# HuaiLeiTang/slam_ros

Hardware: NVIDIA B200
Metric: EKF predict+update steps/s at N landmarks (higher is better)
Workload: dtype f64

## Files before the change

slam_ros_b200/csrc/ekf_kernels.cu:

```cuda
#include "ekf_internal.h"
#include "ekf_device.cuh"
#include <stdlib.h>
#include <string.h>
#include <cuda.h>
#include <cooperative_groups.h>
namespace cg = cooperative_groups;

#define EKF_BLOCK 256

namespace {

__device__ __forceinline__ int owner_of_row(const EkfGeom& g, int r) { return (r / EKF_TILE) % g.world; }
__device__ __forceinline__ size_t local_row(const EkfGeom& g, int r) {
  return (size_t)((r / EKF_TILE) / g.world) * EKF_TILE + (size_t)(r % EKF_TILE);
}
__device__ __forceinline__ bool is_hot(int r, int q) {
  return r <= 2 || q == r || (q == r + 1 && (r & 1));
}
__device__ __forceinline__ double hot_value(const EkfGeom& g, const EkfBuffers& b, int r, int q) {
  if (r <= 2) return b.top[(size_t)r * g.ld + q];
  const int j = (r - 3) >> 1;
  if (r & 1) return b.diag[4 * j + (q - r)];
  return b.diag[4 * j + 2];
}
// ... 319 lines not shown
        d.pa = sub_rank2(d.pa, d.v[t], s_ka[i0 + t]);
        d.pb = sub_rank2(d.pb, d.v[t], s_kb[i0 + t]);
      }
    }
  } else if (d.kind == 2) {
    for (int i0 = 0; i0 < npt; i0 += 8) {
      if (i0 > 0) {
#pragma unroll
        for (int t = 0; t < 8; ++t) if (i0 + t < npt) d.v[t] = b.Kp[(size_t)pl.slot(i0 + t) * g.ld + r];
      }
#pragma unroll
      for (int t = 0; t < 8; ++t) if (i0 + t < npt) {
        d.pa = sub_rank2(d.pa, s_ksa[i0 + t], d.v[t]);
        d.pb = sub_rank2(d.pb, s_ksb[i0 + t], d.v[t]);
      }
    }
  }
}
__device__ __forceinline__ void gain_row_emit(const EkfGeom& g, const EkfBuffers& b, const Gate& G, int r, int out_slot,
                                              const GainRow& d) {
  double2 Kr, KSr;
  gain_row(G, d.p0, d.p1, d.p2, d.pa, d.pb, Kr, KSr);
  b.Kp[(size_t)out_slot * g.ld + r] = Kr;
  b.KSp[(size_t)out_slot * g.ld + r] = KSr;
}

__device__ __forceinline__ double* xchg_col(const EkfPeers& pe, const EkfGeom& g, int p, int par, int which) {
  return pe.xchg[p] + ((size_t)(2 * par + which)) * g.ld;
}
__device__ __forceinline__ unsigned long long* xchg_flags(const EkfPeers& pe, const EkfGeom& g, int p) {
  return reinterpret_cast<unsigned long long*>(pe.xchg[p] + (size_t)4 * g.ld);
}
__device__ __forceinline__ unsigned long long ld_acquire_sys(const unsigned long long* p) {
  unsigned long long v;
  asm volatile("ld.acquire.sys.global.u64 %0, [%1];" : "=l"(v) : "l"(p) : "memory");
  return v;
}
__device__ __forceinline__ void st_relaxed_sys(unsigned long long* p, unsigned long long v) {
  asm volatile("st.relaxed.sys.global.u64 [%0], %1;" ::"l"(p), "l"(v) : "memory");
}
__device__ __forceinline__ void xgpu_exchange_barrier(const EkfPeers& pe, const EkfGeom& g, unsigned long long epoch, int* sticky) {
  __threadfence_system();
  for (int p = 0; p < pe.world; ++p) st_relaxed_sys(xchg_flags(pe, g, p) + pe.rank, epoch);
  const unsigned long long* mine = xchg_flags(pe, g, pe.rank);
  for (int q = 0; q < pe.world; ++q) {
    long long spins = 0;
    while (ld_acquire_sys(mine + q) < epoch) {
      if (++spins > 40000000LL) { atomicOr(sticky, EKF_STICKY_XCHG); break; }
    }
  }
}

#ifdef EKF_LINE_TIMING
__device__ unsigned long long g_line_ts[64 * 16];
__device__ __forceinline__ unsigned long long gtimer() { unsigned long long t; asm volatile("mov.u64 %0, %%globaltimer;" : "=l"(t)); return t; }
#define TS(slot) do { if (gtid == 0 && line - line0 < 64) g_line_ts[(line - line0) * 16 + (slot)] = gtimer(); } while (0)
#else
#define TS(slot) do { } while (0)
#endif

template <int FL_THREADS, bool COOP, bool SHARD>
__global__ void __launch_bounds__(FL_THREADS, FL_THREADS == 256 ? 3 : 1) k_scan_lines(EkfGeom g, EkfBuffers b, const double* __restrict__ z,
                                                              const double* __restrict__ R, int line0, int line1,
                                                              int own_slot0, int prev_slot0, const int* __restrict__ prev_cnt_ptr,
                                                              EkfPeers pe) {
  __shared__ int s_min[FL_THREADS / 32];
  __shared__ double2 s_ka[FL_MAXP], s_kb[FL_MAXP], s_ksa[FL_MAXP], s_ksb[FL_MAXP];
  const int prev_cnt = prev_cnt_ptr ? *prev_cnt_ptr : 0;
  EkfDevState* st = b.st;
  const int gtid = blockIdx.x * blockDim.x + threadIdx.x;
  const int gstride = gridDim.x * blockDim.x;
  auto group_sync = [] () {
    if (COOP) cg::this_grid().sync(); else cg::this_cluster().sync();
  };
  const int L = st->L, nl = 3 + 2 * L, epoch = st->epoch, pbase = st->pbase;
  int nm = b.pidx[line0];
  int ne = b.eidx[line0];
  const int xseq0 = SHARD ? st->xseq : 0;
  int xdone = 0;
  double A[3][3], xp[3];
  load_rr(g, b.top, A);
  xp[0] = st->x_pre[0]; xp[1] = st->x_pre[1]; xp[2] = st->x_pre[2];
  bool have_prev = false;
  int np_prev = 0;
  double pv0 = 0.0, pv1 = 0.0;
  double pS[4] = {0, 0, 0, 0};
  for (int line = line0; line <= line1; ++line) {
    const bool gating = line < line1;
    if (!gating && !have_prev) break;
    TS(0);
    double Rl[4] = {0, 0, 0, 0}, z0 = 0, z1 = 0;
    if (gating) {
      Rl[0] = R[4 * line]; Rl[1] = R[4 * line + 1]; Rl[2] = R[4 * line + 2]; Rl[3] = R[4 * line + 3];
      z0 = z[2 * line]; z1 = z[2 * line + 1];
    }
    const double2* Kv = b.Kp + (size_t)(own_slot0 + np_prev) * g.ld;
    const double2* KSv = b.KSp + (size_t)(own_slot0 + np_prev) * g.ld;
    double2 ks[3], kk[3];
    if (have_prev) {
      for (int r = 0; r < 3; ++r) { ks[r] = KSv[r]; kk[r] = Kv[r]; }
    }
    int cand = EKF_NO_MATCH;
    bool robot_done = !have_prev;
    for (int j = gtid; j < L; j += gstride) {
      const int a = 3 + 2 * j, bb = a + 1;
      double t0a = b.top[a], t0b = b.top[bb];
      double t1a = b.top[(size_t)g.ld + a], t1b = b.top[(size_t)g.ld + bb];
      double t2a = b.top[(size_t)2 * g.ld + a], t2b = b.top[(size_t)2 * g.ld + bb];
      double daa = b.diag[4 * j], dab = b.diag[4 * j + 1], dbb = b.diag[4 * j + 2];
      double ya = b.y[a], yb = b.y[bb];
      const int mt = b.matched[j];
      if (have_prev) {
        const double2 ka = Kv[a], kb = Kv[bb], ksa = KSv[a], ksb = KSv[bb];
        t0a = sub_rank2(t0a, ks[0], ka); t0b = sub_rank2(t0b, ks[0], kb);
        t1a = sub_rank2(t1a, ks[1], ka); t1b = sub_rank2(t1b, ks[1], kb);
        t2a = sub_rank2(t2a, ks[2], ka); t2b = sub_rank2(t2b, ks[2], kb);
        daa = sub_rank2(daa, ksa, ka); dab = sub_rank2(dab, ksa, kb); dbb = sub_rank2(dbb, ksb, kb);
        double ta = 0.0, tb = 0.0;
        axpy_skip(ta, ka.x, pv0); axpy_skip(ta, ka.y, pv1);
        axpy_skip(tb, kb.x, pv0); axpy_skip(tb, kb.y, pv1);
        ya = add_rn(ya, ta); yb = add_rn(yb, tb);
        b.top[a] = t0a; b.top[bb] = t0b;
        b.top[(size_t)g.ld + a] = t1a; b.top[(size_t)g.ld + bb] = t1b;
        b.top[(size_t)2 * g.ld + a] = t2a; b.top[(size_t)2 * g.ld + bb] = t2b;
        b.diag[4 * j] = daa; b.diag[4 * j + 1] = dab; b.diag[4 * j + 2] = dbb;
        b.y[a] = ya; b.y[bb] = yb;
      }
// ... 108 lines not shown
        break;
      }
      const double* cA = xchg_col(pe, g, g.rank, xpar, 0);
      const double* cB = xchg_col(pe, g, g.rank, xpar, 1);
      for (r = gtid; r < nl; r += gstride) {
        GainRow e;
        if (r <= 2) { e.p0 = A[r][0]; e.p1 = A[r][1]; e.p2 = A[r][2]; e.pa = b.top[(size_t)r * g.ld + a]; e.pb = b.top[(size_t)r * g.ld + bb]; }
        else {
          e.p0 = b.top[r]; e.p1 = b.top[(size_t)g.ld + r]; e.p2 = b.top[(size_t)2 * g.ld + r];
          if (r == a) { e.pa = b.diag[4 * j]; e.pb = b.diag[4 * j + 1]; }
          else if (r == bb) { e.pa = b.diag[4 * j + 1]; e.pb = b.diag[4 * j + 2]; }
          else { e.pa = __ldcg(cA + r); e.pb = __ldcg(cB + r); }
        }
        gain_row_emit(g, b, G, r, own_slot0 + np, e);
      }
    }
    if (gtid == 0) {
      b.matched[j] = epoch;
      b.jout[line] = j;
      b.pidx[line + 1] = nm + 1; b.eidx[line + 1] = ne;
      st->np = np + 1;
    }
    TS(6);
    group_sync();
    TS(7);
    have_prev = true;
    np_prev = np;
    nm += 1;
    pv0 = G.v[0]; pv1 = G.v[1];
    for (int t = 0; t < 4; ++t) pS[t] = G.S[t];
  }
  if (SHARD && gtid == 0) st->xseq = xseq0 + xdone;
}

struct HotLm { double t0a, t0b, t1a, t1b, t2a, t2b, daa, dab, dbb, ya, yb; int mt; };
__device__ __forceinline__ void hot_load(const EkfGeom& g, const EkfBuffers& b, int j, HotLm& h) {
  const int a = 3 + 2 * j;
  h.t0a = b.top[a]; h.t0b = b.top[a + 1];
  h.t1a = b.top[(size_t)g.ld + a]; h.t1b = b.top[(size_t)g.ld + a + 1];
  h.t2a = b.top[(size_t)2 * g.ld + a]; h.t2b = b.top[(size_t)2 * g.ld + a + 1];
  h.daa = b.diag[4 * j]; h.dab = b.diag[4 * j + 1]; h.dbb = b.diag[4 * j + 2];
  h.ya = b.y[a]; h.yb = b.y[a + 1];
  h.mt = b.matched[j];
}
__device__ __forceinline__ void hot_store(const EkfGeom& g, const EkfBuffers& b, int j, const HotLm& h) {
  const int a = 3 + 2 * j;
  b.top[a] = h.t0a; b.top[a + 1] = h.t0b;
  b.top[(size_t)g.ld + a] = h.t1a; b.top[(size_t)g.ld + a + 1] = h.t1b;
  b.top[(size_t)2 * g.ld + a] = h.t2a; b.top[(size_t)2 * g.ld + a + 1] = h.t2b;
  b.diag[4 * j] = h.daa; b.diag[4 * j + 1] = h.dab; b.diag[4 * j + 2] = h.dbb;
  b.y[a] = h.ya; b.y[a + 1] = h.yb;
}

template <int FL_THREADS, bool COOP, bool CACHED>
__global__ void __launch_bounds__(FL_THREADS, 1) k_scan_lines2(EkfGeom g, EkfBuffers b, const double* __restrict__ z,
                                                               const double* __restrict__ R, int line0, int line1,
                                                               int own_slot0, int prev_slot0, const int* __restrict__ prev_cnt_ptr,
                                                               const double* __restrict__ pred_u, const double* __restrict__ pred_x, int pred_m,
                                                               const int* __restrict__ pred_carry) {
  __shared__ int s_min[FL_THREADS / 32];
  __shared__ double2 s_ka[FL_MAXP], s_kb[FL_MAXP], s_ksa[FL_MAXP], s_ksb[FL_MAXP];
  const int prev_cnt = prev_cnt_ptr ? *prev_cnt_ptr : 0;
  EkfDevState* st = b.st;
  const int gtid = blockIdx.x * blockDim.x + threadIdx.x;
  const int gstride = gridDim.x * blockDim.x;
  const int scribe = gstride - 1;
  auto group_sync = [] () {
    if (COOP) cg::this_grid().sync(); else cg::this_cluster().sync();
  };
  if (pred_u) {
    predict_body(g, b, pred_u, pred_x, pred_m, gtid, gstride, pred_carry);
    __threadfence();
    group_sync();
  }
  const int L = st->L, epoch = st->epoch, pbase = st->pbase;
  int nm = b.pidx[line0];
  int ne = b.eidx[line0];
  double A[3][3], xp[3];
  load_rr(g, b.top, A);
  xp[0] = st->x_pre[0]; xp[1] = st->x_pre[1]; xp[2] = st->x_pre[2];
  constexpr bool cached = CACHED;
  HotLm h;
  if (cached && gtid < L) hot_load(g, b, gtid, h);
  PendingList pl;
  pl.prev_cnt = prev_cnt; pl.prev_slot0 = prev_slot0; pl.own_slot0 = own_slot0;
  for (int line = line0; line < line1; ++line) {
    TS(0);
    const double Rl[4] = {R[4 * line], R[4 * line + 1], R[4 * line + 2], R[4 * line + 3]};
    const double z0 = z[2 * line], z1 = z[2 * line + 1];
    int cand = EKF_NO_MATCH;
    for (int j = gtid; j < L; j += gstride) {
      if (!cached) hot_load(g, b, j, h);
      if (cand == EKF_NO_MATCH && h.mt != epoch) {
        double Cm[5][5];
        for (int r = 0; r < 3; ++r) for (int q = 0; q < 3; ++q) Cm[r][q] = A[r][q];
        Cm[0][3] = Cm[3][0] = h.t0a; Cm[0][4] = Cm[4][0] = h.t0b;
        Cm[1][3] = Cm[3][1] = h.t1a; Cm[1][4] = Cm[4][1] = h.t1b;
        Cm[2][3] = Cm[3][2] = h.t2a; Cm[2][4] = Cm[4][2] = h.t2b;
        Cm[3][3] = h.daa; Cm[3][4] = Cm[4][3] = h.dab; Cm[4][4] = h.dbb;
        Gate G;
        gate_from_block(Cm, h.ya, h.yb, xp, z0, z1, Rl, G);
        if (G.singular) atomicOr(&st->sticky, EKF_STICKY_SINGULAR);
        else if (!gate_rejects_d2(G.d2, g.gate_d2max)) {
          cand = j;
          double* rec = b.gates + (size_t)GATE_REC * j;
          gate_store(rec, G);
          rec[14] = h.t0a; rec[15] = h.t0b; rec[16] = h.t1a; rec[17] = h.t1b; rec[18] = h.t2a; rec[19] = h.t2b;
        }
      }
    }
    TS(1);
    cand = __reduce_min_sync(0xffffffffu, cand);
    if ((threadIdx.x & 31) == 0) s_min[threadIdx.x >> 5] = cand;
    __syncthreads();
    if (threadIdx.x < 32) {
      int v = (threadIdx.x < FL_THREADS / 32) ? s_min[threadIdx.x] : EKF_NO_MATCH;
      v = __reduce_min_sync(0xffffffffu, v);
      if (threadIdx.x == 0 && v != EKF_NO_MATCH) atomicMin(&b.jbest[line], v);
    }
    TS(2);
    group_sync();
    TS(3);
    const int jw = b.jbest[line];
    const int np = nm - pbase;
    if (jw != EKF_NO_MATCH) TS(8);
    if (jw == EKF_NO_MATCH) {
      if (gtid == scribe) { b.ext[ne] = line; b.eidx[line + 1] = ne + 1; b.pidx[line + 1] = nm; b.jout[line] = -1; }
      ne += 1;
      continue;
    }
    const int aw = 3 + 2 * jw, bw = aw + 1;
    const double* rec = b.gates + (size_t)GATE_REC * jw;
    Gate G;
    gate_load(rec, G);
    TS(9);
    const double wt[3][2] = {{rec[14], rec[15]}, {rec[16], rec[17]}, {rec[18], rec[19]}};
    const int npt = prev_cnt + np;
    for (int i = threadIdx.x; i < npt; i += blockDim.x) {
      const int slot = pl.slot(i);
      s_ka[i] = b.Kp[(size_t)slot * g.ld + aw]; s_kb[i] = b.Kp[(size_t)slot * g.ld + bw];
      s_ksa[i] = b.KSp[(size_t)slot * g.ld + aw]; s_ksb[i] = b.KSp[(size_t)slot * g.ld + bw];
    }
    const int out_slot = own_slot0 + np;
    double2 kk[3], ks[3];
#pragma unroll
    for (int r = 0; r < 3; ++r) gain_row(G, A[r][0], A[r][1], A[r][2], wt[r][0], wt[r][1], kk[r], ks[r]);
    if (gtid == scribe) {
#pragma unroll
      for (int r = 0; r < 3; ++r) { b.Kp[(size_t)out_slot * g.ld + r] = kk[r]; b.KSp[(size_t)out_slot * g.ld + r] = ks[r]; }
    }
    TS(10);
    const double v0 = G.v[0], v1 = G.v[1];
    constexpr int CH = 4;
    const int jc = gtid;
    const bool own1 = cached && jc < L;
    double cpa[2] = {0.0, 0.0}, cpb[2] = {0.0, 0.0};
    double2 cv[2][CH];
    int ckind = 0;
    if (own1 && jc != jw) {
      const int a = 3 + 2 * jc;
      ckind = jc < jw ? 1 : 2;
#pragma unroll
      for (int hf = 0; hf < 2; ++hf) {
        const int r = a + hf;
        if (ckind == 1) { cpa[hf] = b.P[(size_t)r * g.ld + aw]; cpb[hf] = b.P[(size_t)r * g.ld + bw]; }
        else { cpa[hf] = b.P[(size_t)aw * g.ld + r]; cpb[hf] = b.P[(size_t)bw * g.ld + r]; }
        const double2* src = ckind == 1 ? b.KSp : b.Kp;
#pragma unroll
        for (int t = 0; t < CH; ++t) if (t < npt) cv[hf][t] = src[(size_t)pl.slot(t) * g.ld + r];
      }
    }
    TS(11);
    __syncthreads();
    TS(4);
    for (int j = gtid; j < L; j += gstride) {
      const int a = 3 + 2 * j, bb = a + 1;
      double2 Ka, KSa, Kb, KSb;
      if (cached) {
        double pa0 = cpa[0], pb0 = cpb[0], pa1 = cpa[1], pb1 = cpb[1];
        if (j == jw) { pa0 = h.daa; pb0 = h.dab; pa1 = h.dab; pb1 = h.dbb; }
        else {
          const double2* src = ckind == 1 ? b.KSp : b.Kp;
          for (int i0 = 0; i0 < npt; i0 += CH) {
            if (i0 > 0) {
#pragma unroll
              for (int t = 0; t < CH; ++t) if (i0 + t < npt) {
                cv[0][t] = src[(size_t)pl.slot(i0 + t) * g.ld + a]; cv[1][t] = src[(size_t)pl.slot(i0 + t) * g.ld + bb];
              }
            }
#pragma unroll
            for (int t = 0; t < CH; ++t) if (i0 + t < npt) {
              if (ckind == 1) {
                pa0 = sub_rank2(pa0, cv[0][t], s_ka[i0 + t]); pb0 = sub_rank2(pb0, cv[0][t], s_kb[i0 + t]);
                pa1 = sub_rank2(pa1, cv[1][t], s_ka[i0 + t]); pb1 = sub_rank2(pb1, cv[1][t], s_kb[i0 + t]);
              } else {
                pa0 = sub_rank2(pa0, s_ksa[i0 + t], cv[0][t]); pb0 = sub_rank2(pb0, s_ksb[i0 + t], cv[0][t]);
                pa1 = sub_rank2(pa1, s_ksa[i0 + t], cv[1][t]); pb1 = sub_rank2(pb1, s_ksb[i0 + t], cv[1][t]);
              }
            }
          }
        }
        TS(12);
        gain_row(G, h.t0a, h.t1a, h.t2a, pa0, pb0, Ka, KSa);
        gain_row(G, h.t0b, h.t1b, h.t2b, pa1, pb1, Kb, KSb);
      } else {
        hot_load(g, b, j, h);
#pragma unroll
        for (int half = 0; half < 2; ++half) {
          const int r = a + half;
          GainRow d;
          d.p0 = half ? h.t0b : h.t0a; d.p1 = half ? h.t1b : h.t1a; d.p2 = half ? h.t2b : h.t2a;
          d.kind = 0;
          if (j == jw) { d.pa = half ? h.dab : h.daa; d.pb = half ? h.dbb : h.dab; }
          else if (j < jw) {
            const double* Pr = b.P + (size_t)r * g.ld;
            d.pa = Pr[aw]; d.pb = Pr[bw];
            d.kind = 1;
#pragma unroll
            for (int t = 0; t < 8; ++t) if (t < npt) d.v[t] = b.KSp[(size_t)pl.slot(t) * g.ld + r];
          } else {
            d.pa = b.P[(size_t)aw * g.ld + r]; d.pb = b.P[(size_t)bw * g.ld + r];
            d.kind = 2;
#pragma unroll
            for (int t = 0; t < 8; ++t) if (t < npt) d.v[t] = b.Kp[(size_t)pl.slot(t) * g.ld + r];
          }
          gain_row_correct(g, b, r, npt, d, pl, s_ka, s_kb, s_ksa, s_ksb);
          if (half) gain_row(G, d.p0, d.p1, d.p2, d.pa, d.pb, Kb, KSb);
          else gain_row(G, d.p0, d.p1, d.p2, d.pa, d.pb, Ka, KSa);
        }
      }
      TS(13);
      b.Kp[(size_t)out_slot * g.ld + a] = Ka; b.KSp[(size_t)out_slot * g.ld + a] = KSa;
      b.Kp[(size_t)out_slot * g.ld + bb] = Kb; b.KSp[(size_t)out_slot * g.ld + bb] = KSb;
      h.t0a = sub_rank2(h.t0a, ks[0], Ka); h.t0b = sub_rank2(h.t0b, ks[0], Kb);
      h.t1a = sub_rank2(h.t1a, ks[1], Ka); h.t1b = sub_rank2(h.t1b, ks[1], Kb);
      h.t2a = sub_rank2(h.t2a, ks[2], Ka); h.t2b = sub_rank2(h.t2b, ks[2], Kb);
      h.daa = sub_rank2(h.daa, KSa, Ka); h.dab = sub_rank2(h.dab, KSa, Kb); h.dbb = sub_rank2(h.dbb, KSb, Kb);
      double ta = 0.0, tb = 0.0;
      axpy_skip(ta, Ka.x, v0); axpy_skip(ta, Ka.y, v1);
      axpy_skip(tb, Kb.x, v0); axpy_skip(tb, Kb.y, v1);
      h.ya = add_rn(h.ya, ta); h.yb = add_rn(h.yb, tb);
      if (j == jw) { h.mt = epoch; b.matched[j] = epoch; }
      hot_store(g, b, j, h);
    }
    TS(5);
    update_robot_block(kk, ks, v0, v1, A, xp);
    if (gtid == scribe) {
      for (int r = 0; r < 3; ++r) {
        for (int q = r; q < 3; ++q) b.top[(size_t)r * g.ld + q] = A[r][q];
        b.y[r] = xp[r]; st->pose[r] = xp[r]; st->x_pre[r] = xp[r];
      }
      st->v[0] = v0; st->v[1] = v1;
      for (int t = 0; t < 4; ++t) st->S[t] = G.S[t];
      b.jout[line] = jw;
      b.pidx[line + 1] = nm + 1; b.eidx[line + 1] = ne;
      st->np = np + 1;
    }
    TS(6);
    nm += 1;
  }
}

__global__ void k_flush_done(EkfBuffers b, int next_line) {
  if (blockIdx.x == 0 && threadIdx.x == 0) { b.st->pbase = b.pidx[next_line]; b.st->np = 0; }
}

__global__ void k_chunk_mark(EkfBuffers b, int next_line, EkfScanView* view) {
  if (blockIdx.x == 0 && threadIdx.x == 0) {
    EkfDevState* st = b.st;
    view->cnt = b.pidx[next_line] - st->pbase; view->L = st->L;
    st->pbase = b.pidx[next_line]; st->np = 0;
  }
}

__global__ void k_queue_all(EkfGeom g, EkfBuffers b, int m) {
  const int gid = blockIdx.x * blockDim.x + threadIdx.x;
  for (int i = gid; i < m; i += gridDim.x * blockDim.x) {
    b.ext[i] = i; b.eidx[i + 1] = i + 1; b.pidx[i + 1] = 0; b.jout[i] = -1;
  }
}

struct TileId { int k, rb, cb; };

__device__ __forceinline__ long long tiles_before(int T, int rank, int world, long long k) {
  return k * (long long)(T - rank) - (long long)world * k * (k - 1) / 2;
}
__device__ __forceinline__ TileId decode_tile(int T, int rank, int world, long long idx) {
  const double A = (double)(T - rank) + 0.5 * world;
  double disc = A * A - 2.0 * world * (double)idx;
  if (disc < 0.0) disc = 0.0;
  long long k = (long long)((A - sqrt(disc)) / world);
  if (k < 0) k = 0;
  while (tiles_before(T, rank, world, k + 1) <= idx) ++k;
  while (k > 0 && tiles_before(T, rank, world, k) > idx) --k;
  TileId t;
  t.k = (int)k;
  t.rb = rank + world * (int)k;
  t.cb = t.rb + (int)(idx - tiles_before(T, rank, world, k));
  return t;
}

template <int C>
__global__ void __launch_bounds__(EKF_BLOCK, 2) k_sweep(EkfGeom g, EkfBuffers b, const int* __restrict__ np_ptr) {
  const int np = np_ptr ? *np_ptr : b.st->np;
  if (np <= 0) return;
  const int nl = 3 + 2 * b.st->L;
  const int T = (nl + EKF_TILE - 1) / EKF_TILE;
  if (g.rank >= T) return;
  const long long K_rows = (T - g.rank + g.world - 1) / g.world;
  const long long total = tiles_before(T, g.rank, g.world, K_rows);
  const long long idx = blockIdx.x;
  if (idx >= total) return;
  const TileId t = decode_tile(T, g.rank, g.world, idx);
// ... 413 lines not shown
    for (int mb = 0; mb < 2; ++mb)
#pragma unroll
      for (int nb = 0; nb < 8; ++nb)
        acc[mb][nb] = *reinterpret_cast<const double2*>(&st.P[(nb * TR + row0 + 8 * mb) * 8 + 2 * tq]);
    if (split) {
      __syncwarp();
      if (lane == 0) mbar_arrive(&sh.emptyP[s]);
    }
    const double* KSw = reinterpret_cast<const double*>(&st.KS[0][0]);
    const double* Kw = reinterpret_cast<const double*>(&st.K[0][0]);
#pragma unroll 2
    for (int k0 = 0; k0 < np; k0 += 2) {
      const int term = k0 + tsel;
      const bool valid = term < np;
      double a[2], bq[8];
#pragma unroll
      for (int mb = 0; mb < 2; ++mb) a[mb] = valid ? -KSw[(term * TR + row0 + 8 * mb) * 2 + comp] : 0.0;
#pragma unroll
      for (int nb = 0; nb < 8; ++nb) bq[nb] = valid ? Kw[(term * TC + 8 * nb + gq) * 2 + comp] : 0.0;
#pragma unroll
      for (int mb = 0; mb < 2; ++mb)
#pragma unroll
        for (int nb = 0; nb < 8; ++nb) dmma884(acc[mb][nb].x, acc[mb][nb].y, a[mb], bq[nb]);
    }
    __syncwarp();
    if (lane == 0) mbar_arrive(&sh.empty[s]);
    double* Pt = dst + ((size_t)lrow0 + row0) * g.ld + (size_t)col0 + 2 * tq;
    if (grow0 + TR <= nl && col0 + TC <= nl) {
#pragma unroll
      for (int mb = 0; mb < 2; ++mb)
#pragma unroll
        for (int nb = 0; nb < 8; ++nb) __stcs(reinterpret_cast<double2*>(Pt + (size_t)(8 * mb) * g.ld + 8 * nb), acc[mb][nb]);
    } else {
#pragma unroll
      for (int mb = 0; mb < 2; ++mb) {
        if (grow0 + row0 + 8 * mb < nl) {
          double* Pr = Pt + (size_t)(8 * mb) * g.ld;
#pragma unroll
          for (int nb = 0; nb < 8; ++nb) {
            const int q = col0 + 8 * nb + 2 * tq;
            if (q + 1 < nl) __stcs(reinterpret_cast<double2*>(Pr + 8 * nb), acc[mb][nb]); else if (q < nl) Pr[8 * nb] = acc[mb][nb].x;
          }
        }
      }
    }
  }
}

__global__ void __launch_bounds__(512) k_end_scan_a(EkfGeom g, EkfBuffers b, const double* __restrict__ z, const double* __restrict__ R, int m,
                                                    int slot0, EkfScanView* view, int prev_slot0, const int* __restrict__ prev_cnt_ptr) {
  EkfDevState* st = b.st;
  __shared__ double s_pose[3];
  __shared__ double s_y01[2];
  if (threadIdx.x == 0) {
    if (m == 0 || b.pidx[m] == 0) {
      b.y[0] = st->x_pre[0]; b.y[1] = st->x_pre[1]; b.y[2] = st->x_pre[2];
      double th = st->x_pre[2];
      normalize_radian(th);
      st->pose[0] = st->x_pre[0]; st->pose[1] = st->x_pre[1]; st->pose[2] = th;
    }
    s_pose[0] = st->pose[0]; s_pose[1] = st->pose[1]; s_pose[2] = st->pose[2];
    s_y01[0] = b.y[0]; s_y01[1] = b.y[1];
  }
  __syncthreads();
  const int ne = b.eidx[m];
  const int L = st->L;
  const int n_add = min(ne, g.cap - L);
  if (threadIdx.x == 0 && blockIdx.x == 0) {
    st->n_added = n_add;
    if (n_add < ne) atomicOr(&st->sticky, EKF_STICKY_CAPACITY);
  }
  {
    const int cnt = b.pidx[m] - st->pbase, r0 = 3 + 2 * L, r1 = 3 + 2 * (L + n_add);
    const int pcnt = prev_cnt_ptr ? *prev_cnt_ptr : 0;
    for (int i = 0; i < cnt + pcnt; ++i) {
      const size_t slot = i < cnt ? slot0 + i : prev_slot0 + (i - cnt);
      for (int r = r0 + threadIdx.x; r < r1; r += blockDim.x) {
        b.Kp[slot * g.ld + r] = make_double2(0.0, 0.0);
        b.KSp[slot * g.ld + r] = make_double2(0.0, 0.0);
      }
    }
  }
  double A[3][3];
  load_rr(g, b.top, A);
  for (int e = blockIdx.x * blockDim.x + threadIdx.x; e < n_add; e += gridDim.x * blockDim.x) {
    const int i = b.ext[e];
    double alfa = z[2 * i], r = z[2 * i + 1];
    const double Rl[4] = {R[4 * i], R[4 * i + 1], R[4 * i + 2], R[4 * i + 3]};
    const int l = 3 + 2 * (L + e);
    r = add_rn(r, add_rn(mul_rn(s_pose[0], cos(alfa)), mul_rn(s_pose[1], sin(alfa))));
    alfa = add_rn(alfa, s_pose[2]);
    double cw, sw;
    cos_sin(alfa, cw, sw);
    const double Gx[2][3] = {{0.0, 0.0, 1.0}, {cw, sw, 0.0}};
    const double Gl[2][2] = {{1.0, 0.0}, {sub_rn(mul_rn(s_y01[1], cw), mul_rn(s_y01[0], sw)), 1.0}};
    normalize_radian(alfa);
    b.y[l] = alfa; b.y[l + 1] = r;
    b.ext_cs[2 * e] = cw; b.ext_cs[2 * e + 1] = sw;
    double GP[2][3] = {{0, 0, 0}, {0, 0, 0}};
    for (int k = 0; k < 3; ++k)
      for (int ii = 0; ii < 2; ++ii) {
        const double t = mul_rn(1.0, Gx[ii][k]);
        if (t != 0.0) for (int jj = 0; jj < 3; ++jj) GP[ii][jj] = add_rn(GP[ii][jj], mul_rn(t, A[k][jj]));
      }
    double Pll[2][2];
    for (int ii = 0; ii < 2; ++ii)
      for (int jj = 0; jj < 2; ++jj) {
        double t = 0.0;
        for (int k = 0; k < 3; ++k) t = add_rn(t, mul_rn(GP[ii][k], Gx[jj][k]));
        Pll[ii][jj] = add_rn(0.0, mul_rn(1.0, t));
      }
    double GR[2][2] = {{0, 0}, {0, 0}};
    for (int k = 0; k < 2; ++k)
      for (int ii = 0; ii < 2; ++ii) {
        const double t = mul_rn(1.0, Gl[ii][k]);
        if (t != 0.0) for (int jj = 0; jj < 2; ++jj) GR[ii][jj] = add_rn(GR[ii][jj], mul_rn(t, Rl[k * 2 + jj]));
      }
    for (int ii = 0; ii < 2; ++ii)
      for (int jj = 0; jj < 2; ++jj) {
        double t = 0.0;
        for (int k = 0; k < 2; ++k) t = add_rn(t, mul_rn(GR[ii][k], Gl[jj][k]));
        Pll[ii][jj] = add_rn(Pll[ii][jj], add_rn(0.0, mul_rn(1.0, t)));
      }
    b.diag[4 * (L + e)] = Pll[0][0]; b.diag[4 * (L + e) + 1] = Pll[0][1]; b.diag[4 * (L + e) + 2] = Pll[1][1];
    b.diag[4 * (L + e) + 3] = 0.0;
    for (int k = 0; k < 3; ++k) {
      double r0 = 0.0, r1 = 0.0;
      for (int kk = 0; kk < 3; ++kk) {
        axpy_skip(r0, mul_rn(1.0, Gx[0][kk]), A[kk][k]);
        axpy_skip(r1, mul_rn(1.0, Gx[1][kk]), A[kk][k]);
      }
      b.top[(size_t)k * g.ld + l] = r0;
      b.top[(size_t)k * g.ld + l + 1] = r1;
    }
  }
  __syncthreads();
  if (threadIdx.x == 0) {
    st->L0 = L;
    int Ln = L + n_add;
    const bool reset = Ln > g.cap - g.headroom;
    if (reset) { Ln = 0; st->resets += 1; }
    st->L = Ln;
    if (view) { view->cnt = reset ? 0 : b.pidx[m] - st->pbase; view->L = Ln; }
  }
}

__global__ void __launch_bounds__(EKF_BLOCK) k_end_scan_b(EkfGeom g, EkfBuffers b, double* __restrict__ P2) {
  const EkfDevState* st = b.st;
  const int n_add = st->n_added;
  const int L = st->L0;
  const int c_idx = blockIdx.x * blockDim.x + threadIdx.x;
  if (c_idx >= 2 * n_add) return;
  const int e = c_idx >> 1, tsel = c_idx & 1;
  const int l = 3 + 2 * (L + e);
  const int col = l + tsel;
  const double cw = b.ext_cs[2 * e], sw = b.ext_cs[2 * e + 1];
  const double* t0p = b.top; const double* t1p = b.top + g.ld; const double* t2p = b.top + 2 * (size_t)g.ld;
  for (int k = 3 + blockIdx.y; k < l; k += gridDim.y) {
    if (g.world > 1 && owner_of_row(g, k) != g.rank) continue;
    double v;
    if (tsel == 0) { v = 0.0; axpy_skip(v, 1.0, t2p[k]); }
    else { v = 0.0; axpy_skip(v, cw, t0p[k]); axpy_skip(v, sw, t1p[k]); }
    b.P[local_row(g, k) * g.ld + col] = v;
    if (P2) P2[local_row(g, k) * g.ld + col] = v;
  }
}

__global__ void __launch_bounds__(EKF_BLOCK) k_assemble(EkfGeom g, EkfBuffers b, int r0, int nr, int c0, int nc,
                                                        double* __restrict__ out, int ld_out) {
  const int nl = 3 + 2 * b.st->L;
  const long long total = (long long)nr * nc;
  for (long long t = blockIdx.x * (long long)blockDim.x + threadIdx.x; t < total;
       t += (long long)gridDim.x * blockDim.x) {
    const int r = r0 + (int)(t / nc), q = c0 + (int)(t % nc);
    double v = 0.0;
    if (r < nl && q < nl) {
      const int lo = min(r, q), hi = max(r, q);
      if (is_hot(lo, hi)) { if (g.rank == 0) v = hot_value(g, b, lo, hi); }
      else if (g.world == 1 || owner_of_row(g, lo) == g.rank) v = b.P[local_row(g, lo) * g.ld + hi];
    }
    out[(size_t)(r - r0) * ld_out + (q - c0)] = v;
  }
}

__global__ void __launch_bounds__(EKF_BLOCK) k_scatter(EkfGeom g, EkfBuffers b, int r0, int nr, int nl,
                                                       const double* __restrict__ in, int ld_in) {
  const long long total = (long long)nr * nl;
  for (long long t = blockIdx.x * (long long)blockDim.x + threadIdx.x; t < total;
       t += (long long)gridDim.x * blockDim.x) {
    const int r = r0 + (int)(t / nl), q = (int)(t % nl);
    if (q < r) continue;
    const double v = in[(size_t)(r - r0) * ld_in + q];
    if (r <= 2) b.top[(size_t)r * g.ld + q] = v;
    else if (is_hot(r, q)) {
      const int j = (r - 3) >> 1;
      if (r & 1) b.diag[4 * j + (q - r)] = v; else b.diag[4 * j + 2] = v;
    } else if (g.world == 1 || owner_of_row(g, r) == g.rank) b.P[local_row(g, r) * g.ld + q] = v;
  }
}

__global__ void __launch_bounds__(EKF_BLOCK) k_cov_rows(EkfGeom g, EkfBuffers b, double* __restrict__ partials) {
  __shared__ double s_sum[EKF_BLOCK], s_sq[EKF_BLOCK];
  const int nl = 3 + 2 * b.st->L;
  for (int r = blockIdx.x; r < nl; r += gridDim.x) {
    double sum = 0.0, sq = 0.0;
    for (int q = threadIdx.x; q < nl; q += blockDim.x) {
      const int lo = min(r, q), hi = max(r, q);
      double v = 0.0;
      if (is_hot(lo, hi)) { if (g.rank == 0) v = hot_value(g, b, lo, hi); }
      else if (g.world == 1 || owner_of_row(g, lo) == g.rank) v = b.P[local_row(g, lo) * g.ld + hi];
      sum += v; sq += v * v;
    }
    s_sum[threadIdx.x] = sum; s_sq[threadIdx.x] = sq;
    __syncthreads();
    for (int w = EKF_BLOCK / 2; w > 0; w >>= 1) {
      if (threadIdx.x < w) { s_sum[threadIdx.x] += s_sum[threadIdx.x + w]; s_sq[threadIdx.x] += s_sq[threadIdx.x + w]; }
      __syncthreads();
    }
// ... 202 lines not shown
  }
}

__global__ void __launch_bounds__(EKF_BLOCK) k_pose_term2(EkfGeom g, EkfBuffers b, int d, const double2* __restrict__ K2,
                                                          const double2* __restrict__ KS2) {
  const bool on = d == 3 && b.st->fix_status == EKF_FIX_ACCEPTED;
  const int gid = blockIdx.x * blockDim.x + threadIdx.x;
  if (gid == 0) b.st->np = on ? 1 : 0;
  if (!on) return;
  const int nl = 3 + 2 * b.st->L;
  for (int r = gid; r < nl; r += gridDim.x * blockDim.x) { b.Kp[r] = K2[r]; b.KSp[r] = KS2[r]; }
}

inline int blocks_for(long long n, int cap = 1 << 20) {
  long long bl = (n + EKF_BLOCK - 1) / EKF_BLOCK;
  if (bl < 1) bl = 1;
  if (bl > cap) bl = cap;
  return (int)bl;
}

}

cudaError_t ekf_launch_init(const EkfGeom& g, const EkfBuffers& b, cudaStream_t s) {
  k_init<<<1, 32, 0, s>>>(g, b);
  return cudaGetLastError();
}
cudaError_t ekf_launch_predict(const EkfGeom& g, const EkfBuffers& b, const double* d_u, const double* d_x_t0,
                               int m, int L_ub, cudaStream_t s, const int* carry) {
  const int work = (3 + 2 * L_ub > m) ? 3 + 2 * L_ub : m;
  k_predict<<<blocks_for(work, 1024), EKF_BLOCK, 0, s>>>(g, b, d_u, d_x_t0, m, carry);
  return cudaGetLastError();
}
cudaError_t ekf_launch_associate(const EkfGeom& g, const EkfBuffers& b, const double* d_z, const double* d_R,
                                 int line, int L_ub, cudaStream_t s) {
  if (L_ub <= 0) return cudaSuccess;
  k_associate<<<blocks_for(L_ub), EKF_BLOCK, 0, s>>>(g, b, d_z, d_R, line);
  return cudaGetLastError();
}
cudaError_t ekf_launch_gain(const EkfGeom& g, const EkfBuffers& b, const double* d_z, const double* d_R,
                            int line, int j_override, int mode, int L_ub, int max_batch, cudaStream_t s) {
  if (L_ub <= 0) return cudaSuccess;
  k_gain<<<blocks_for(3 + 2 * L_ub, 2048), EKF_BLOCK, 0, s>>>(g, b, d_z, d_R, line, j_override, mode, max_batch);
  return cudaGetLastError();
}
cudaError_t ekf_launch_apply(const EkfGeom& g, const EkfBuffers& b, int line, int j_override, int L_ub,
                             cudaStream_t s) {
  k_apply<<<blocks_for(3 + 2 * L_ub, 2048), EKF_BLOCK, 0, s>>>(g, b, line, j_override);
  return cudaGetLastError();
}
#ifdef EKF_LINE_TIMING
extern "C" int ekf_debug_line_timing(unsigned long long* out, int n) {
  return (int)cudaMemcpyFromSymbol(out, g_line_ts, sizeof(unsigned long long) * (size_t)n);
}
#endif
void ekf_prefer_max_smem_carveout(void) {
  const int c = cudaSharedmemCarveoutMaxShared;
  cudaFuncSetAttribute(k_predict, cudaFuncAttributePreferredSharedMemoryCarveout, c);
  cudaFuncSetAttribute(k_scan_lines<512, true, false>, cudaFuncAttributePreferredSharedMemoryCarveout, c);
  cudaFuncSetAttribute(k_scan_lines<512, true, true>, cudaFuncAttributePreferredSharedMemoryCarveout, c);
  cudaFuncSetAttribute(k_scan_lines<512, false, false>, cudaFuncAttributePreferredSharedMemoryCarveout, c);
  cudaFuncSetAttribute(k_scan_lines2<512, true, true>, cudaFuncAttributePreferredSharedMemoryCarveout, c);
  cudaFuncSetAttribute(k_scan_lines2<512, true, false>, cudaFuncAttributePreferredSharedMemoryCarveout, c);
  cudaFuncSetAttribute(k_scan_lines2<512, false, true>, cudaFuncAttributePreferredSharedMemoryCarveout, c);
  cudaFuncSetAttribute(k_scan_lines2<256, false, true>, cudaFuncAttributePreferredSharedMemoryCarveout, c);
  cudaFuncSetAttribute(k_scan_lines2<512, false, false>, cudaFuncAttributePreferredSharedMemoryCarveout, c);
  cudaFuncSetAttribute(k_end_scan_a, cudaFuncAttributePreferredSharedMemoryCarveout, c);
  cudaFuncSetAttribute(k_end_scan_b, cudaFuncAttributePreferredSharedMemoryCarveout, c);
  cudaFuncSetAttribute(k_chunk_mark, cudaFuncAttributePreferredSharedMemoryCarveout, c);
  cudaFuncSetAttribute(k_queue_all, cudaFuncAttributePreferredSharedMemoryCarveout, c);
  (void)cudaGetLastError();
}
static int line_loop_v1() { static int v = -1; if (v < 0) { const char* e = getenv("EKF_LINE_LOOP"); v = (e && atoi(e) == 1) ? 1 : 0; } return v; }
int ekf_pick_cluster(void) {
  cudaFuncSetAttribute(k_scan_lines<512, false, false>, cudaFuncAttributeNonPortableClusterSizeAllowed, 1);
  cudaFuncSetAttribute(k_scan_lines2<512, false, true>, cudaFuncAttributeNonPortableClusterSizeAllowed, 1);
  cudaFuncSetAttribute(k_scan_lines2<256, false, true>, cudaFuncAttributeNonPortableClusterSizeAllowed, 1);
  cudaFuncSetAttribute(k_scan_lines2<512, false, false>, cudaFuncAttributeNonPortableClusterSizeAllowed, 1);
  { const char* e = getenv("EKF_CLUSTER"); const int v = e ? atoi(e) : 0; if (v == 1 || v == 2 || v == 4 || v == 8) return v; }
  const int tries[2] = {16, 8};
  for (int t = 0; t < 2; ++t) {
    cudaLaunchConfig_t cfg;
    memset(&cfg, 0, sizeof cfg);
    cfg.gridDim = dim3(tries[t]); cfg.blockDim = dim3(512);
    cudaLaunchAttribute attr[1];
    attr[0].id = cudaLaunchAttributeClusterDimension;
    attr[0].val.clusterDim.x = tries[t]; attr[0].val.clusterDim.y = 1; attr[0].val.clusterDim.z = 1;
    cfg.attrs = attr; cfg.numAttrs = 1;
    int n = 0;
    int n2 = 0;
    if (cudaOccupancyMaxActiveClusters(&n, k_scan_lines<512, false, false>, &cfg) == cudaSuccess && n >= 1 &&
        cudaOccupancyMaxActiveClusters(&n2, k_scan_lines2<512, false, false>, &cfg) == cudaSuccess && n2 >= 1) return tries[t];
  }
  (void)cudaGetLastError();
  return 8;
}
int ekf_scan_lines_fuses_predict(const EkfPeers* peers) { return !line_loop_v1() && !(peers && peers->world > 1); }
cudaError_t ekf_launch_scan_lines(const EkfGeom& g, const EkfBuffers& b, const double* d_z, const double* d_R,
                                  int line0, int line1, int ctas, int coop, int own_slot0, int prev_slot0,
                                  const int* prev_cnt_ptr, const EkfPeers* peers, int L_ub, cudaStream_t s,
                                  const double* pred_u, const double* pred_x, int pred_m, const int* pred_carry) {
  if (line1 <= line0) return cudaSuccess;
  if (pred_u && !ekf_scan_lines_fuses_predict(peers)) return cudaErrorInvalidValue;
  EkfPeers pe;
  memset(&pe, 0, sizeof pe);
  pe.world = 1;
  if (peers) pe = *peers;
  if (coop) {
    void* args[] = {(void*)&g, (void*)&b, (void*)&d_z, (void*)&d_R, (void*)&line0, (void*)&line1, (void*)&own_slot0,
                    (void*)&prev_slot0, (void*)&prev_cnt_ptr, (void*)&pe};
    if (peers && peers->world > 1)
      return cudaLaunchCooperativeKernel((const void*)k_scan_lines<512, true, true>, dim3(ctas), dim3(512), args, 0, s);
    if (line_loop_v1())
      return cudaLaunchCooperativeKernel((const void*)k_scan_lines<512, true, false>, dim3(ctas), dim3(512), args, 0, s);
    void* args2[] = {(void*)&g, (void*)&b, (void*)&d_z, (void*)&d_R, (void*)&line0, (void*)&line1, (void*)&own_slot0,
                     (void*)&prev_slot0, (void*)&prev_cnt_ptr, (void*)&pred_u, (void*)&pred_x, (void*)&pred_m, (void*)&pred_carry};
    static int lt = -1;
    if (lt < 0) { const char* e = getenv("EKF_LINE_THREADS"); lt = e ? atoi(e) : 0; }
    if (L_ub > g.cap) L_ub = g.cap;
    if (lt == 256 && L_ub <= ctas * 256)
      return cudaLaunchCooperativeKernel((const void*)k_scan_lines2<256, true, true>, dim3(ctas), dim3(256), args2, 0, s);
    if (L_ub <= ctas * 512) return cudaLaunchCooperativeKernel((const void*)k_scan_lines2<512, true, true>, dim3(ctas), dim3(512), args2, 0, s);
    return cudaLaunchCooperativeKernel((const void*)k_scan_lines2<512, true, false>, dim3(ctas), dim3(512), args2, 0, s);
  }
  cudaLaunchConfig_t cfg;
  memset(&cfg, 0, sizeof cfg);
  cfg.gridDim = dim3(ctas); cfg.blockDim = dim3(512); cfg.dynamicSmemBytes = 0; cfg.stream = s;
  cudaLaunchAttribute attr[1];
  attr[0].id = cudaLaunchAttributeClusterDimension;
  attr[0].val.clusterDim.x = ctas; attr[0].val.clusterDim.y = 1; attr[0].val.clusterDim.z = 1;
  cfg.attrs = attr; cfg.numAttrs = 1;
  if (line_loop_v1())
    return cudaLaunchKernelEx(&cfg, k_scan_lines<512, false, false>, g, b, d_z, d_R, line0, line1, own_slot0, prev_slot0, prev_cnt_ptr, pe);
  if (L_ub <= ctas * 256) {
    cfg.blockDim = dim3(256);
    return cudaLaunchKernelEx(&cfg, k_scan_lines2<256, false, true>, g, b, d_z, d_R, line0, line1, own_slot0, prev_slot0, prev_cnt_ptr, pred_u, pred_x, pred_m, pred_carry);
  }
  if (L_ub <= ctas * 512)
    return cudaLaunchKernelEx(&cfg, k_scan_lines2<512, false, true>, g, b, d_z, d_R, line0, line1, own_slot0, prev_slot0, prev_cnt_ptr, pred_u, pred_x, pred_m, pred_carry);
  return cudaLaunchKernelEx(&cfg, k_scan_lines2<512, false, false>, g, b, d_z, d_R, line0, line1, own_slot0, prev_slot0, prev_cnt_ptr, pred_u, pred_x, pred_m, pred_carry);
}
cudaError_t ekf_launch_flush_done(const EkfBuffers& b, int next_line, cudaStream_t s) {
  k_flush_done<<<1, 32, 0, s>>>(b, next_line);
  return cudaGetLastError();
}
cudaError_t ekf_launch_chunk_mark(const EkfBuffers& b, int next_line, EkfScanView* view, cudaStream_t s) {
  k_chunk_mark<<<1, 32, 0, s>>>(b, next_line, view);
  return cudaGetLastError();
}
cudaError_t ekf_launch_queue_all(const EkfGeom& g, const EkfBuffers& b, int m, cudaStream_t s) {
  if (m <= 0) return cudaSuccess;
  k_queue_all<<<blocks_for(m, 1024), EKF_BLOCK, 0, s>>>(g, b, m);
  return cudaGetLastError();
}
int ekf_sweep_grid_ub(const EkfGeom& g, int L_ub) {
  const int nl = 3 + 2 * L_ub;
  const int T = (nl + EKF_TILE - 1) / EKF_TILE;
  if (g.rank >= T) return 0;
  const long long K = (T - g.rank + g.world - 1) / g.world;
  const long long total = K * (long long)(T - g.rank) - (long long)g.world * K * (K - 1) / 2;
  return (int)total;
}
cudaError_t ekf_launch_sweep(const EkfGeom& g, const EkfBuffers& b, const int* np_ptr, int np_ub, int L_ub,
                             cudaStream_t s) {
  const int grid = ekf_sweep_grid_ub(g, L_ub);
  if (grid <= 0 || np_ub <= 0) return cudaSuccess;
  if (np_ub <= 1) k_sweep<1><<<grid, EKF_BLOCK, 0, s>>>(g, b, np_ptr);
  else if (np_ub <= 2) k_sweep<2><<<grid, EKF_BLOCK, 0, s>>>(g, b, np_ptr);
  else if (np_ub <= 4) k_sweep<4><<<grid, EKF_BLOCK, 0, s>>>(g, b, np_ptr);
  else k_sweep<8><<<grid, EKF_BLOCK, 0, s>>>(g, b, np_ptr);
  return cudaGetLastError();
}
template <int TR, int TC, int STAGES, int CW, int C>
static cudaError_t launch_sweep_shape(const EkfGeom& g, const EkfBuffers& b, const CUtensorMap* m, const CUtensorMap* mK,
                                      const CUtensorMap* mKS, double* dst, int slot0,
// ... 223 lines not shown
```

Measured before the change: 3174.

## Prefetch pending K rows through a cp.async shared-memory ring in line scan

Adds a per-thread shared-memory ring (12 slots of 32 bytes) filled with cp.async so the pending KSp/Kp column pairs for a thread's landmark are loaded ahead of the rank-2 correction loop, instead of being read from global memory in chunks. It also adds a device-side pick kernel that chooses the cached or uncached body from the actual landmark count rather than the host upper bound. Both paths are on by default through environment switches. In exchange the kernel uses about 192 KB of dynamic shared memory per block, adds per-slot async-wait latency, and the change carries extra timing instrumentation under a debug macro.

```diff
diff --git a/slam_ros_b200/csrc/ekf_kernels.cu b/slam_ros_b200/csrc/ekf_kernels.cu
--- a/slam_ros_b200/csrc/ekf_kernels.cu
+++ b/slam_ros_b200/csrc/ekf_kernels.cu
@@ -395,11 +395,19 @@
 }
 
 #ifdef EKF_LINE_TIMING
-__device__ unsigned long long g_line_ts[64 * 16];
+#define EKF_TS_SCANS 32
+__device__ unsigned long long g_line_ts[EKF_TS_SCANS * 64 * 16];
+__device__ unsigned long long g_scan_ts[EKF_TS_SCANS * 8];
+__device__ unsigned g_ts_scan;
 __device__ __forceinline__ unsigned long long gtimer() { unsigned long long t; asm volatile("mov.u64 %0, %%globaltimer;" : "=l"(t)); return t; }
-#define TS(slot) do { if (gtid == 0 && line - line0 < 64) g_line_ts[(line - line0) * 16 + (slot)] = gtimer(); } while (0)
+#define TS(slot) do { if (gtid == 0 && line - line0 < 64) g_line_ts[(ts_scan * 64 + line - line0) * 16 + (slot)] = gtimer(); } while (0)
+#define TS_VAL(slot, v) do { if (gtid == 0 && line - line0 < 64) g_line_ts[(ts_scan * 64 + line - line0) * 16 + (slot)] = (unsigned long long)(v); } while (0)
+#define TS_SCAN_NO(s) const unsigned ts_scan = (s) % EKF_TS_SCANS
+#define TS_SCAN(slot) (g_scan_ts[ts_scan * 8 + (slot)] = gtimer())
 #else
 #define TS(slot) do { } while (0)
+#define TS_VAL(slot, v) do { } while (0)
+#define TS_SCAN_NO(s) do { } while (0)
 #endif
 
 template <int FL_THREADS, bool COOP, bool SHARD>
@@ -416,6 +424,7 @@
   auto group_sync = [] () {
     if (COOP) cg::this_grid().sync(); else cg::this_cluster().sync();
   };
+  TS_SCAN_NO(0);
   const int L = st->L, nl = 3 + 2 * L, epoch = st->epoch, pbase = st->pbase;
   int nm = b.pidx[line0];
   int ne = b.eidx[line0];
@@ -630,12 +639,20 @@
   b.y[a] = h.ya; b.y[a + 1] = h.yb;
 }
 
-template <int FL_THREADS, bool COOP, bool CACHED>
-__global__ void __launch_bounds__(FL_THREADS, 1) k_scan_lines2(EkfGeom g, EkfBuffers b, const double* __restrict__ z,
-                                                               const double* __restrict__ R, int line0, int line1,
-                                                               int own_slot0, int prev_slot0, const int* __restrict__ prev_cnt_ptr,
-                                                               const double* __restrict__ pred_u, const double* __restrict__ pred_x, int pred_m,
-                                                               const int* __restrict__ pred_carry) {
+#define FL_RING 12
+__device__ __forceinline__ void cp_async16(void* dst, const void* src) {
+  asm volatile("cp.async.cg.shared.global [%0], [%1], 16;" ::"r"((unsigned)__cvta_generic_to_shared(dst)), "l"(src) : "memory");
+}
+__device__ __forceinline__ void cp_async_commit() { asm volatile("cp.async.commit_group;" ::: "memory"); }
+template <int N>
+__device__ __forceinline__ void cp_async_wait() { asm volatile("cp.async.wait_group %0;" ::"n"(N) : "memory"); }
+
+template <int FL_THREADS, bool COOP, bool CACHED, int RING>
+__device__ __forceinline__ void scan_lines2_body(EkfGeom g, EkfBuffers b, const double* __restrict__ z,
+                                                 const double* __restrict__ R, int line0, int line1,
+                                                 int own_slot0, int prev_slot0, const int* __restrict__ prev_cnt_ptr,
+                                                 const double* __restrict__ pred_u, const double* __restrict__ pred_x, int pred_m,
+                                                 const int* __restrict__ pred_carry) {
   __shared__ int s_min[FL_THREADS / 32];
   __shared__ double2 s_ka[FL_MAXP], s_kb[FL_MAXP], s_ksa[FL_MAXP], s_ksb[FL_MAXP];
   const int prev_cnt = prev_cnt_ptr ? *prev_cnt_ptr : 0;
@@ -646,12 +663,26 @@
   auto group_sync = [] () {
     if (COOP) cg::this_grid().sync(); else cg::this_cluster().sync();
   };
+  static_assert(RING == 0 || CACHED, "the ring holds the rows of the thread's one landmark");
+  extern __shared__ double2 s_ring[];
+  double2* my_ring = s_ring + 2 * threadIdx.x;
+#ifdef EKF_LINE_TIMING
+  TS_SCAN_NO(g_ts_scan);
+  if (gtid == 0) {
+    for (int i = 0; i < 8; ++i) g_scan_ts[ts_scan * 8 + i] = 0;
+    for (int i = 0; i < 64 * 16; ++i) g_line_ts[ts_scan * 64 * 16 + i] = 0;
+    TS_SCAN(0);
+  }
+#endif
   if (pred_u) {
     predict_body(g, b, pred_u, pred_x, pred_m, gtid, gstride, pred_carry);
     __threadfence();
     group_sync();
   }
   const int L = st->L, epoch = st->epoch, pbase = st->pbase;
+#ifdef EKF_LINE_TIMING
+  if (gtid == 0) { TS_SCAN(1); g_scan_ts[ts_scan * 8 + 7] = (unsigned long long)(long long)pbase; }
+#endif
   int nm = b.pidx[line0];
   int ne = b.eidx[line0];
   double A[3][3], xp[3];
@@ -714,6 +745,7 @@
     TS(9);
     const double wt[3][2] = {{rec[14], rec[15]}, {rec[16], rec[17]}, {rec[18], rec[19]}};
     const int npt = prev_cnt + np;
+    TS_VAL(14, npt); TS_VAL(15, CACHED ? 1 : 2);
     for (int i = threadIdx.x; i < npt; i += blockDim.x) {
       const int slot = pl.slot(i);
       s_ka[i] = b.Kp[(size_t)slot * g.ld + aw]; s_kb[i] = b.Kp[(size_t)slot * g.ld + bw];
@@ -744,8 +776,21 @@
         if (ckind == 1) { cpa[hf] = b.P[(size_t)r * g.ld + aw]; cpb[hf] = b.P[(size_t)r * g.ld + bw]; }
         else { cpa[hf] = b.P[(size_t)aw * g.ld + r]; cpb[hf] = b.P[(size_t)bw * g.ld + r]; }
         const double2* src = ckind == 1 ? b.KSp : b.Kp;
-#pragma unroll
-        for (int t = 0; t < CH; ++t) if (t < npt) cv[hf][t] = src[(size_t)pl.slot(t) * g.ld + r];
+        if (!RING) {
+#pragma unroll
+          for (int t = 0; t < CH; ++t) if (t < npt) cv[hf][t] = src[(size_t)pl.slot(t) * g.ld + r];
+        }
+      }
+      if (RING) {
+        const double2* src = (ckind == 1 ? b.KSp : b.Kp) + a;
+#pragma unroll
+        for (int t = 0; t < RING; ++t) {
+          if (t < npt) {
+            const double2* q = src + (size_t)pl.slot(t) * g.ld;
+            cp_async16(my_ring + t * 2 * FL_THREADS, q); cp_async16(my_ring + t * 2 * FL_THREADS + 1, q + 1);
+          }
+          cp_async_commit();
+        }
       }
     }
     TS(11);
@@ -759,7 +804,25 @@
         if (j == jw) { pa0 = h.daa; pb0 = h.dab; pa1 = h.dab; pb1 = h.dbb; }
         else {
           const double2* src = ckind == 1 ? b.KSp : b.Kp;
-          for (int i0 = 0; i0 < npt; i0 += CH) {
+          if (RING) {
+            for (int i = 0, sl = 0; i < npt; ++i) {
+              cp_async_wait<(RING > 0 ? RING - 1 : 0)>();
+              const double2 c0 = my_ring[sl * 2 * FL_THREADS], c1 = my_ring[sl * 2 * FL_THREADS + 1];
+              if (ckind == 1) {
+                pa0 = sub_rank2(pa0, c0, s_ka[i]); pb0 = sub_rank2(pb0, c0, s_kb[i]);
+                pa1 = sub_rank2(pa1, c1, s_ka[i]); pb1 = sub_rank2(pb1, c1, s_kb[i]);
+              } else {
+                pa0 = sub_rank2(pa0, s_ksa[i], c0); pb0 = sub_rank2(pb0, s_ksb[i], c0);
+                pa1 = sub_rank2(pa1, s_ksa[i], c1); pb1 = sub_rank2(pb1, s_ksb[i], c1);
+              }
+              if (i + RING < npt) {
+                const double2* q = src + (size_t)pl.slot(i + RING) * g.ld + a;
+                cp_async16(my_ring + sl * 2 * FL_THREADS, q); cp_async16(my_ring + sl * 2 * FL_THREADS + 1, q + 1);
+              }
+              cp_async_commit();
+              sl = sl + 1 == RING ? 0 : sl + 1;
+            }
+          } else for (int i0 = 0; i0 < npt; i0 += CH) {
             if (i0 > 0) {
 #pragma unroll
               for (int t = 0; t < CH; ++t) if (i0 + t < npt) {
@@ -837,6 +900,34 @@
     TS(6);
     nm += 1;
   }
+#ifdef EKF_LINE_TIMING
+  if (threadIdx.x == 0) atomicMax(&g_scan_ts[ts_scan * 8 + 2], gtimer());
+  if (gtid == 0) g_ts_scan += 1;
+#endif
+}
+
+template <int FL_THREADS, bool COOP, bool CACHED, int RING = 0>
+__global__ void __launch_bounds__(FL_THREADS, 1) k_scan_lines2(EkfGeom g, EkfBuffers b, const double* __restrict__ z,
+                                                               const double* __restrict__ R, int line0, int line1,
+                                                               int own_slot0, int prev_slot0, const int* __restrict__ prev_cnt_ptr,
+                                                               const double* __restrict__ pred_u, const double* __restrict__ pred_x, int pred_m,
+                                                               const int* __restrict__ pred_carry) {
+  scan_lines2_body<FL_THREADS, COOP, CACHED, RING>(g, b, z, R, line0, line1, own_slot0, prev_slot0, prev_cnt_ptr, pred_u, pred_x,
+                                                   pred_m, pred_carry);
+}
+
+template <int RING>
+__global__ void __launch_bounds__(512, 1) k_scan_lines2_pick(EkfGeom g, EkfBuffers b, const double* __restrict__ z,
+                                                            const double* __restrict__ R, int line0, int line1,
+                                                            int own_slot0, int prev_slot0, const int* __restrict__ prev_cnt_ptr,
+                                                            const double* __restrict__ pred_u, const double* __restrict__ pred_x, int pred_m,
+                                                            const int* __restrict__ pred_carry) {
+  if (b.st->L <= (int)(gridDim.x * 512))
+    scan_lines2_body<512, true, true, RING>(g, b, z, R, line0, line1, own_slot0, prev_slot0, prev_cnt_ptr, pred_u, pred_x,
+                                            pred_m, pred_carry);
+  else
+    scan_lines2_body<512, true, false, 0>(g, b, z, R, line0, line1, own_slot0, prev_slot0, prev_cnt_ptr, pred_u, pred_x,
+                                          pred_m, pred_carry);
 }
 
 __global__ void k_flush_done(EkfBuffers b, int next_line) {
@@ -1356,6 +1447,10 @@
   EkfDevState* st = b.st;
   __shared__ double s_pose[3];
   __shared__ double s_y01[2];
+#ifdef EKF_LINE_TIMING
+  TS_SCAN_NO(g_ts_scan + EKF_TS_SCANS - 1);
+  if (threadIdx.x == 0) TS_SCAN(3);
+#endif
   if (threadIdx.x == 0) {
     if (m == 0 || b.pidx[m] == 0) {
       b.y[0] = st->x_pre[0]; b.y[1] = st->x_pre[1]; b.y[2] = st->x_pre[2];
@@ -1446,6 +1541,9 @@
     if (reset) { Ln = 0; st->resets += 1; }
     st->L = Ln;
     if (view) { view->cnt = reset ? 0 : b.pidx[m] - st->pbase; view->L = Ln; }
+#ifdef EKF_LINE_TIMING
+    TS_SCAN(4);
+#endif
   }
 }
 
@@ -1454,6 +1552,11 @@
   const int n_add = st->n_added;
   const int L = st->L0;
   const int c_idx = blockIdx.x * blockDim.x + threadIdx.x;
+#ifdef EKF_LINE_TIMING
+  TS_SCAN_NO(g_ts_scan + EKF_TS_SCANS - 1);
+  if (threadIdx.x == 0 && blockIdx.x == 0 && blockIdx.y == 0) TS_SCAN(5);
+  if (threadIdx.x == 0) atomicMax(&g_scan_ts[ts_scan * 8 + 6], gtimer());
+#endif
   if (c_idx >= 2 * n_add) return;
   const int e = c_idx >> 1, tsel = c_idx & 1;
   const int l = 3 + 2 * (L + e);
@@ -1468,6 +1571,9 @@
     b.P[local_row(g, k) * g.ld + col] = v;
     if (P2) P2[local_row(g, k) * g.ld + col] = v;
   }
+#ifdef EKF_LINE_TIMING
+  if (threadIdx.x == 0) atomicMax(&g_scan_ts[ts_scan * 8 + 6], gtimer());
+#endif
 }
 
 __global__ void __launch_bounds__(EKF_BLOCK) k_assemble(EkfGeom g, EkfBuffers b, int r0, int nr, int c0, int nc,
@@ -1776,6 +1882,11 @@
 extern "C" int ekf_debug_line_timing(unsigned long long* out, int n) {
   return (int)cudaMemcpyFromSymbol(out, g_line_ts, sizeof(unsigned long long) * (size_t)n);
 }
+extern "C" int ekf_debug_scan_timing(unsigned long long* out, unsigned* nscan) {
+  cudaError_t e = cudaMemcpyFromSymbol(out, g_scan_ts, sizeof(g_scan_ts));
+  if (e == cudaSuccess) e = cudaMemcpyFromSymbol(nscan, g_ts_scan, sizeof(unsigned));
+  return (int)e;
+}
 #endif
 void ekf_prefer_max_smem_carveout(void) {
   const int c = cudaSharedmemCarveoutMaxShared;
@@ -1784,6 +1895,13 @@
   cudaFuncSetAttribute(k_scan_lines<512, true, true>, cudaFuncAttributePreferredSharedMemoryCarveout, c);
   cudaFuncSetAttribute(k_scan_lines<512, false, false>, cudaFuncAttributePreferredSharedMemoryCarveout, c);
   cudaFuncSetAttribute(k_scan_lines2<512, true, true>, cudaFuncAttributePreferredSharedMemoryCarveout, c);
+  cudaFuncSetAttribute(k_scan_lines2<512, true, true, FL_RING>, cudaFuncAttributePreferredSharedMemoryCarveout, c);
+  cudaFuncSetAttribute(k_scan_lines2<512, true, true, FL_RING>, cudaFuncAttributeMaxDynamicSharedMemorySize,
+                       (int)(FL_RING * 512 * 2 * sizeof(double2)));
+  cudaFuncSetAttribute(k_scan_lines2_pick<FL_RING>, cudaFuncAttributePreferredSharedMemoryCarveout, c);
+  cudaFuncSetAttribute(k_scan_lines2_pick<FL_RING>, cudaFuncAttributeMaxDynamicSharedMemorySize,
+                       (int)(FL_RING * 512 * 2 * sizeof(double2)));
+  cudaFuncSetAttribute(k_scan_lines2_pick<0>, cudaFuncAttributePreferredSharedMemoryCarveout, c);
   cudaFuncSetAttribute(k_scan_lines2<512, true, false>, cudaFuncAttributePreferredSharedMemoryCarveout, c);
   cudaFuncSetAttribute(k_scan_lines2<512, false, true>, cudaFuncAttributePreferredSharedMemoryCarveout, c);
   cudaFuncSetAttribute(k_scan_lines2<256, false, true>, cudaFuncAttributePreferredSharedMemoryCarveout, c);
@@ -1843,7 +1961,18 @@
     if (L_ub > g.cap) L_ub = g.cap;
     if (lt == 256 && L_ub <= ctas * 256)
       return cudaLaunchCooperativeKernel((const void*)k_scan_lines2<256, true, true>, dim3(ctas), dim3(256), args2, 0, s);
-    if (L_ub <= ctas * 512) return cudaLaunchCooperativeKernel((const void*)k_scan_lines2<512, true, true>, dim3(ctas), dim3(512), args2, 0, s);
+    const char* er = getenv("EKF_LINE_RING");
+    const char* ep = getenv("EKF_LINE_PICK");
+    const bool ring = !(er && atoi(er) == 0), pick = !(ep && atoi(ep) == 0);
+    const size_t ring_bytes = ring ? (size_t)FL_RING * 512 * 2 * sizeof(double2) : 0;
+    if (L_ub <= ctas * 512) {
+      if (!ring) return cudaLaunchCooperativeKernel((const void*)k_scan_lines2<512, true, true>, dim3(ctas), dim3(512), args2, 0, s);
+      return cudaLaunchCooperativeKernel((const void*)k_scan_lines2<512, true, true, FL_RING>, dim3(ctas), dim3(512), args2,
+                                         ring_bytes, s);
+    }
+    if (pick)
+      return cudaLaunchCooperativeKernel(ring ? (const void*)k_scan_lines2_pick<FL_RING> : (const void*)k_scan_lines2_pick<0>,
+                                         dim3(ctas), dim3(512), args2, ring_bytes, s);
     return cudaLaunchCooperativeKernel((const void*)k_scan_lines2<512, true, false>, dim3(ctas), dim3(512), args2, 0, s);
   }
   cudaLaunchConfig_t cfg;
```

Result: no change. 3175, median of 6 (+0.0%).
